# GAP-LAB-CUHK-SZ/gaustudio

Measured on AMD Instinct MI355X. Metric: Mpixels/s fwd+bwd @1M Gaussians 1920x1080, higher is better.
Workload: dtype f32; 1 GPU; C3: 1M synthetic Gaussians, 1920x1080, SH degree 3, fwd+bwd (colour+depth+median+opacity consumed); gaussians=1000000, width=1920, height=1080, sh_degree=3, tiles=8160, views_per_rank=1, loss=colour + depth + median + opacity gradients consumed, camera=static (the same view every step), parallelism=single GPU

## Files before the change

### gaustudio_amd/csrc/gsr_kernels_bwd.hip

```cpp
#include "gsr_internal.h"
#include "gsr_bwd_timing.h"

namespace gsr {

__device__ __constant__ float bSH_C0 = 0.28209479177387814f;
__device__ __constant__ float bSH_C1 = 0.4886025119029199f;
__device__ __constant__ float bSH_C2[5] = {1.0925484305920792f, -1.0925484305920792f, 0.31539156525252005f,
                                            -1.0925484305920792f, 0.5462742152960396f};
__device__ __constant__ float bSH_C3[7] = {-0.5900435899266435f, 2.890611442640554f, -0.4570457994644658f,
                                            0.3731763325901154f, -0.4570457994644658f, 1.445305721320277f,
                                            -0.5900435899266435f};

#define GSR_DPP_ADD(v, ctrl) v += __int_as_float(__builtin_amdgcn_update_dpp(0, __float_as_int(v), ctrl, 0xF, 0xF, true))
#define GSR_DPP_OF(v, ctrl) __int_as_float(__builtin_amdgcn_update_dpp(0, __float_as_int(v), ctrl, 0xF, 0xF, true))
__device__ __forceinline__ float half_swap_sum(float a, float b)
{
	const auto t = __builtin_amdgcn_permlane32_swap(__float_as_uint(a), __float_as_uint(b), false, false);
	return __uint_as_float(t[0]) + __uint_as_float(t[1]);
}
__device__ __forceinline__ float row_swap_sum(float p, float q)
{
	const auto t = __builtin_amdgcn_permlane16_swap(__float_as_uint(p), __float_as_uint(q), false, false);
	return __uint_as_float(t[0]) + __uint_as_float(t[1]);
}
// ... 194 lines not shown
	const bool any_bg = __ballot(bg_dot != 0.f) != 0ull;
	float T_ = T_final;
	float S = 0.f;

	int wmax = lc;
#pragma unroll
	for (int o = 32; o > 0; o >>= 1) wmax = max(wmax, __shfl_xor(wmax, o, 64));
	wmax = __builtin_amdgcn_readfirstlane(wmax);
	if (lane == 0) s_max[wv] = wmax;
	__syncthreads();
	const int bmax = max(max(s_max[0], s_max[1]), max(s_max[2], s_max[3]));

	for (int i = bmax + tid; !FLAGS && i < (int)(range.y - range.x); i += GSR_BWD_THREADS) {
		const uint32_t id = point_list[range.x + i];
		const uint4 q3 = recs[id].q3;
		float4* dst = reinterpret_cast<float4*>(rows + (size_t)(goff[id] + gs_row_in_rect(q3.x, q3.y, (q3.z >> GSR_Q3Z_DEAD_SHIFT) & 15u, tx, ty)) * GSR_ROW_STRIDE);
		dst[0] = make_float4(0.f, 0.f, 0.f, 0.f);
		dst[1] = make_float4(0.f, 0.f, 0.f, 0.f);
		dst[2] = make_float4(0.f, 0.f, 0.f, 0.f);
	}
	float2* slab = s_slab[wv];
	float* plane = s_plane[wv];
	const int srec = tid >> 2, spart = tid & 3;
	auto load_id = [&](int t) -> uint32_t {
		return (t > 0 && srec < min(GSR_BWD_BATCH, t)) ? point_list[range.x + (uint32_t)(t - 1 - srec)] : 0u;
	};
	auto load_part = [&](int t, uint32_t id) -> float4 {
		float4 v = make_float4(0.f, 0.f, 0.f, 0.f);
		if (t > 0 && srec < min(GSR_BWD_BATCH, t)) {
			v = reinterpret_cast<const float4*>(recs + id)[spart];
			if (spart == 3) v.w = __uint_as_float(goff[id]);
		}
		return v;
	};
	uint32_t id_next = load_id(bmax - GSR_BWD_BATCH);
	float4 part_cur = load_part(bmax, load_id(bmax));
	for (int top = bmax; top > 0; top -= GSR_BWD_BATCH) {
		const int cnt = min(GSR_BWD_BATCH, top);
		__syncthreads();
		if (srec < cnt) {
			if (spart == 0) sA[srec] = part_cur;
			else if (spart == 1) sB[srec] = part_cur;
			else if (spart == 2) sC[srec] = part_cur;
			else {
				const uint32_t q3x = __float_as_uint(part_cur.x), q3y = __float_as_uint(part_cur.y), q3w = __float_as_uint(part_cur.w);
				s_row[srec] = q3w + gs_row_in_rect(q3x, q3y, (__float_as_uint(part_cur.z) >> GSR_Q3Z_DEAD_SHIFT) & 15u, tx, ty);
			}
		}
		const float4 part_next = load_part(top - GSR_BWD_BATCH, id_next);
		id_next = load_id(top - 2 * GSR_BWD_BATCH);
		for (int i = tid; i < 4 * GSR_BWD_BATCH * GSR_PLANE_STRIDE / 4; i += GSR_BWD_THREADS)
			reinterpret_cast<float4*>(&s_plane[0][0])[i] = make_float4(0.f, 0.f, 0.f, 0.f);
		__syncthreads();
		bool hit = false;
		if (lane < cnt && top - 1 - lane < wmax) hit = gs_box_may_touch(sA[lane], sB[lane], fbx, fby, bx1, by1);
		unsigned long long m = __ballot(hit);
		int nu = 0;
		unsigned long long unit_js = 0ull;
		auto pair = [&](const float4 A, const float4 B, const float4 Cc, const int j) {
			const int pos = top - 1 - j;
			const float dx = A.x - pixfx, dy = A.y - pixfy;
			const float power = FMA(A.w * dx, dy, FMA(B.x * dy, dy, (A.z * dx) * dx));
			const float G = gs_exp(power);
			const float a0 = B.y * G;
			const bool live = (pos < lc) & (power <= 0.0f) & (power >= B.w) & (!(a0 < 1.0f / 255.0f));
			if (__ballot(live) == 0ull) return;
			const float Gm = live ? G : 0.f;
			const float alpha = fminf(0.99f, B.y * Gm);
			const float rinv = __builtin_amdgcn_rcpf(1.0f - alpha);
			const float test_T = T_ * rinv;
			const float w = alpha * test_T;
			const float cd = FMA(Cc.x, dLp0, FMA(Cc.y, dLp1, FMA(Cc.z, dLp2, FMA(B.z, dLd, dLo))));
			const float diff = cd - S;
			float dL_dalpha = diff * test_T;
			if (any_bg) {
				asm volatile("");
				dL_dalpha = FMA(-(T_final * rinv), bg_dot, dL_dalpha);
			}
			const float q = Gm * dL_dalpha;
			S = FMA(alpha, diff, S);
			T_ = TSEL ? (live ? test_T : T_) : test_T;
			slab[nu * GSR_SLAB_STRIDE + lane] = make_float2(q, w);
			unit_js |= (unsigned long long)j << (8 * nu);
			nu++;
			if (nu == GSR_BWD_UNITS) {
				__builtin_amdgcn_fence(__ATOMIC_RELEASE, "wavefront");
				__builtin_amdgcn_wave_barrier();
				gs_bwd_phase2(GSR_BWD_UNITS, slab, unit_js, sA, s_tab[wv], fbx, fby, top, plane, lane);
				__builtin_amdgcn_wave_barrier();
				nu = 0;
				unit_js = 0ull;
			}
		};
		if (m) {
			int j0 = __ffsll((long long)m) - 1, j1 = 0;
			m &= m - 1;
			float4 A0 = sA[j0], B0 = sB[j0], C0 = sC[j0], A1, B1, C1;
			while (true) {
				const bool more1 = m != 0ull;
				if (more1) {
					j1 = __ffsll((long long)m) - 1;
					m &= m - 1;
					A1 = sA[j1]; B1 = sB[j1]; C1 = sC[j1];
				}
				pair(A0, B0, C0, j0);
				if (!more1) break;
				const bool more0 = m != 0ull;
				if (more0) {
					j0 = __ffsll((long long)m) - 1;
					m &= m - 1;
					A0 = sA[j0]; B0 = sB[j0]; C0 = sC[j0];
				}
				pair(A1, B1, C1, j1);
				if (!more0) break;
			}
		}
		if (nu > 0) {
			__builtin_amdgcn_fence(__ATOMIC_RELEASE, "wavefront");
			__builtin_amdgcn_wave_barrier();
			gs_bwd_phase2(nu, slab, unit_js, sA, s_tab[wv], fbx, fby, top, plane, lane);
		}
		__syncthreads();
		if (tid < cnt) {
			float v[10];
#pragma unroll
			for (int k = 0; k < 10; k++)
				v[k] = ((s_plane[0][tid * GSR_PLANE_STRIDE + k] + s_plane[1][tid * GSR_PLANE_STRIDE + k]) +
				        s_plane[2][tid * GSR_PLANE_STRIDE + k]) + s_plane[3][tid * GSR_PLANE_STRIDE + k];
			const float4 A = sA[tid], B = sB[tid];
			const float ca = -2.f * A.z, cb = -A.w, cc = -2.f * B.x, op = B.y;
			const float M10 = v[0], M01 = v[1], M20 = v[2], M11 = v[3], M02 = v[4];
			const float ddelx_dx = (float)(0.5 * W), ddely_dy = (float)(0.5 * H);
			const uint32_t my_row = s_row[tid];
			float4* dst = reinterpret_cast<float4*>(rows + (size_t)my_row * GSR_ROW_STRIDE);
			dst[0] = make_float4(-(op * FMA(cb, M01, ca * M10)) * ddelx_dx, -(op * FMA(cb, M10, cc * M01)) * ddely_dy,
			                     -0.5f * op * M20, -0.5f * op * M11);
			dst[1] = make_float4(-0.5f * op * M02, v[5], v[6], v[7]);
			dst[2] = make_float4(v[8], v[9], 0.f, 0.f);
			if (FLAGS) row_flags[my_row] = 1;
		}
		part_cur = part_next;
	}
}

#endif

#define GSR_BWQ_U 4
#ifndef GSR_BWQ_BATCH
#define GSR_BWQ_BATCH 128
#endif
#define GSR_BWQ_HALVES ((GSR_BWQ_BATCH + 63) / 64)
#define GSR_BWQ_LIST (GSR_BWQ_BATCH + 8)
#define GSR_BWQ_SENT GSR_BWQ_BATCH
#define GSR_WAIT_VM0() __builtin_amdgcn_s_waitcnt(0x0F70)
#define GSR_BWQ_QSTRIDE 66

#ifndef GSR_BWQ_WAVES
#define GSR_BWQ_WAVES 4
#endif
template <bool FLAGS, bool TSEL, bool FX, bool CONLY>
__global__ __launch_bounds__(GSR_BWD_THREADS) __attribute__((amdgpu_waves_per_eu(GSR_BWQ_WAVES, GSR_BWQ_WAVES))) void composite_bwd_quarter_kernel(
    int T, int chunk, int gx, int W, int H, const GsBg bgv, const uint2* __restrict__ ranges,
    const uint32_t* __restrict__ point_list, const GsRec* __restrict__ recs, const uint32_t* __restrict__ goff,
    const float* __restrict__ final_T, const uint32_t* __restrict__ n_contrib, const uint32_t* __restrict__ med_pos,
    const float* __restrict__ dL_dpix, const float* __restrict__ dL_dpix_depth, const float* __restrict__ dL_dpix_median,
    const float* __restrict__ dL_dpix_opacity, float* __restrict__ rows, uint8_t* __restrict__ row_flags,
    const GsCtl* __restrict__ ctl)
{
	__shared__ float4 sA[GSR_BWQ_BATCH + 1];
	__shared__ float4 sB[GSR_BWQ_BATCH + 1];
	__shared__ float4 sC[GSR_BWQ_BATCH + 1];
	__shared__ uint32_t s_row[GSR_BWQ_BATCH];
	__shared__ uint16_t s_qmask[GSR_BWQ_BATCH];
	__shared__ __attribute__((aligned(16))) float s_plane[4][GSR_BWQ_BATCH * GSR_PLANE_STRIDE];
	__shared__ __attribute__((aligned(16))) float2 s_slab[4][4 * GSR_BWQ_QSTRIDE];
	__shared__ __attribute__((aligned(16))) uint8_t s_list[4][4][GSR_BWQ_LIST];
	__shared__ int s_max[4];
	if (blockIdx.x == 0 && threadIdx.x == 0 && bgv.flag_dst != nullptr) *bgv.flag_dst = bgv.flag;
	const int tb_lo = (int)bgv.tile_lo, tb_n = (int)min(bgv.tile_hi, (uint32_t)T) - tb_lo;
	const int local = (blockIdx.x & 7) * chunk + (blockIdx.x >> 3);
	const int tile = bgv.tile_order ? ((int)blockIdx.x < T ? (int)bgv.tile_order[blockIdx.x] : T) : tb_lo + local;
	if ((!bgv.tile_order && ((int)(blockIdx.x >> 3) >= chunk || local >= tb_n)) || tile >= T) return;
	if ((uint32_t)tile < bgv.tile_lo || (uint32_t)tile >= bgv.tile_hi) return;
	const int tid = threadIdx.x;
	const int lane = tid & 63, wv = tid >> 6, qd = lane >> 4;
	TM_DECL
	const int tx = tile % gx, ty = tile / gx;
	const int lx = ((wv & 1) << 3) + ((qd & 1) << 2) + (lane & 3);
	const int ly = ((wv >> 1) << 3) + ((qd >> 1) << 2) + ((lane >> 2) & 3);
	const int px = tx * GSR_BLOCK_X + lx, py = ty * GSR_BLOCK_Y + ly;
	const bool inside = px < W && py < H;
	const float pixfx = (float)px, pixfy = (float)py;
	const float fbx = (float)(tx * GSR_BLOCK_X + ((wv & 1) << 3)), fby = (float)(ty * GSR_BLOCK_Y + ((wv >> 1) << 3));
	const uint2 range = ranges[tile];
	const bool have_qmask = __builtin_amdgcn_readfirstlane(ctl->has_qmask) != 0u;
	const uint16_t* __restrict__ qmask = gs_qmask_ptr(point_list, __builtin_amdgcn_readfirstlane(ctl->num_binned));

	const size_t sidx = (size_t)tile * GSR_TILE_PIX + (wv << 6) + ((ly & 7) << 3) + (lx & 7);
	const float T_final = inside ? final_T[sidx] : 0.f;
	const int lc = inside ? (int)n_contrib[sidx] : 0;
	float dLp0 = 0.f, dLp1 = 0.f, dLp2 = 0.f, dLd = 0.f, dLo = 0.f, dLm = 0.f;
	uint32_t mpos = 0u;
	if (inside) {
		const size_t HW = (size_t)H * W;
		const size_t pix_id = (size_t)W * py + px;
		if (dL_dpix) {
			dLp0 = dL_dpix[pix_id];
			dLp1 = dL_dpix[HW + pix_id];
			dLp2 = dL_dpix[2 * HW + pix_id];
		}
		if (!CONLY) {
			if (dL_dpix_depth) dLd = dL_dpix_depth[pix_id];
			if (dL_dpix_median) dLm = dL_dpix_median[pix_id];
			if (dL_dpix_opacity) dLo = dL_dpix_opacity[pix_id];
			mpos = med_pos[sidx];
		}
	}
	float2* slab = s_slab[wv];
	float* plane = s_plane[wv];
	const int u2 = (lane >> 2) & 3, r2 = lane & 3;
	float4 g_pix[4];
	float g_op[4];
	{
		float4* tmp = reinterpret_cast<float4*>(slab);
		tmp[2 * lane] = make_float4(dLp0, dLp1, dLp2, dLd);
		if (!CONLY) tmp[2 * lane + 1] = make_float4(dLo, 0.f, 0.f, 0.f);
		__builtin_amdgcn_fence(__ATOMIC_RELEASE, "wavefront");
		__builtin_amdgcn_wave_barrier();
#pragma unroll
		for (int sx = 0; sx < 4; sx++) {
			const int pl = (qd << 4) + (r2 << 2) + sx;
			const float4 gp = tmp[2 * pl];
			const float c0 = gp.x, c1 = gp.y, c2 = gp.z, c3 = gp.w;
			g_pix[sx] = make_float4(r2 == 0 ? c0 : r2 == 1 ? c1 : r2 == 2 ? c2 : c3, r2 == 0 ? c1 : r2 == 1 ? c0 : r2 == 2 ? c3 : c2,
			                        r2 == 0 ? c2 : r2 == 1 ? c3 : r2 == 2 ? c0 : c1, r2 == 0 ? c3 : r2 == 1 ? c2 : r2 == 2 ? c1 : c0);
			g_op[sx] = CONLY ? 0.f : tmp[2 * pl + 1].x;
		}
		__builtin_amdgcn_wave_barrier();
#pragma unroll
		for (int sx = 0; sx < 4; sx++) asm volatile("" : "+v"(g_pix[sx].x), "+v"(g_pix[sx].y), "+v"(g_pix[sx].z), "+v"(g_pix[sx].w));
	}
	const float y2 = fby + (float)(((qd >> 1) << 2) + r2), x2 = fbx + (float)((qd & 1) << 2);
	const float bg0 = bgv.dptr ? bgv.dptr[0] : bgv.host[0], bg1 = bgv.dptr ? bgv.dptr[1] : bgv.host[1], bg2 = bgv.dptr ? bgv.dptr[2] : bgv.host[2];
	const float bg_dot = FMA(bg2, dLp2, FMA(bg1, dLp1, FMA(bg0, dLp0, 0.f)));
	const bool any_bg = __ballot(bg_dot != 0.f) != 0ull;
	float T_ = T_final;
	float S = 0.f;

	int qmax = lc;
	qmax = max(qmax, __shfl_xor(qmax, 1, 64));
	qmax = max(qmax, __shfl_xor(qmax, 2, 64));
	qmax = max(qmax, __shfl_xor(qmax, 4, 64));
	qmax = max(qmax, __shfl_xor(qmax, 8, 64));
	const int qm0 = __builtin_amdgcn_readlane(qmax, 0), qm1 = __builtin_amdgcn_readlane(qmax, 16);
	const int qm2 = __builtin_amdgcn_readlane(qmax, 32), qm3 = __builtin_amdgcn_readlane(qmax, 48);
	const int wmax = max(max(qm0, qm1), max(qm2, qm3));
	if (lane == 0) s_max[wv] = wmax;
	TM(0)
	if (tid < 3) (tid == 0 ? sA : tid == 1 ? sB : sC)[GSR_BWQ_SENT] = make_float4(0.f, 0.f, 0.f, 0.f);
	__syncthreads();
	const int bmax = max(max(s_max[0], s_max[1]), max(s_max[2], s_max[3]));
	TM(1)

	const int srec = tid >> 2, spart = tid & 3;
	const uint32_t* __restrict__ tile_list = point_list + range.x;
	const uint32_t* __restrict__ mask_words = have_qmask ? reinterpret_cast<const uint32_t*>(qmask) : point_list;
	auto list_pos = [&](int t, int h) -> uint32_t {
		return (uint32_t)max(t - 1 - (srec + 64 * h), 0);
	};
	auto word_ptr = [&](int t, int h, uint32_t id) -> const uint32_t* {
		return spart == 2 ? mask_words + ((range.x + list_pos(t, h)) >> 1) : goff + id;
	};
	uint32_t id_next[GSR_BWQ_HALVES];
	float4 part[GSR_BWQ_HALVES];
#pragma unroll
	for (int h = 0; h < GSR_BWQ_HALVES; h++) {
		part[h] = make_float4(0.f, 0.f, 0.f, 0.f);
		id_next[h] = 0u;
	}
	if (bmax > 0) {
		uint32_t id_cur[GSR_BWQ_HALVES];
#pragma unroll
		for (int h = 0; h < GSR_BWQ_HALVES; h++) {
			id_cur[h] = tile_list[list_pos(bmax, h)];
			id_next[h] = tile_list[list_pos(bmax - GSR_BWQ_BATCH, h)];
		}
#pragma unroll
		for (int h = 0; h < GSR_BWQ_HALVES; h++) {
			part[h] = reinterpret_cast<const float4*>(recs + id_cur[h])[spart];
			if (spart >= 2) part[h].w = __uint_as_float(*word_ptr(bmax, h, id_cur[h]));
		}
	}
	for (int i = bmax + tid; !FLAGS && i < (int)(range.y - range.x); i += GSR_BWD_THREADS) {
		const uint32_t id = tile_list[i];
		const uint4 q3 = recs[id].q3;
		float4* dst = reinterpret_cast<float4*>(rows + (size_t)(goff[id] + gs_row_in_rect(q3.x, q3.y, (q3.z >> GSR_Q3Z_DEAD_SHIFT) & 15u, tx, ty)) * GSR_ROW_STRIDE);
		dst[0] = make_float4(0.f, 0.f, 0.f, 0.f);
		dst[1] = make_float4(0.f, 0.f, 0.f, 0.f);
		dst[2] = make_float4(0.f, 0.f, 0.f, 0.f);
	}
	GSR_WAIT_VM0();
	TM(2)
	const uint8_t* my_list = &s_list[wv][qd][0];
	const char* recA = reinterpret_cast<const char*>(sA);
	const char* recB = reinterpret_cast<const char*>(sB);
	const char* recC = reinterpret_cast<const char*>(sC);
	float2* my_slab_w = slab + qd * GSR_BWQ_QSTRIDE + (lane & 15);
	const float4* my_slab_r = reinterpret_cast<const float4*>(slab + qd * GSR_BWQ_QSTRIDE + u2 * 16 + r2 * 4);

	for (int top = bmax; top > 0; top -= GSR_BWQ_BATCH) {
		const int cnt = min(GSR_BWQ_BATCH, top);
		TM(3)
		__syncthreads();
		TM(4)
#pragma unroll
		for (int h = 0; h < GSR_BWQ_HALVES; h++) {
			const int sr = srec + 64 * h;
			if (sr < cnt) {
				if (spart == 0) sA[sr] = part[h];
				else if (spart == 1) {
					float* b = reinterpret_cast<float*>(&sB[sr]);
					*reinterpret_cast<float2*>(b) = make_float2(part[h].x, part[h].y);
					b[2] = part[h].z;
					reinterpret_cast<float2*>(&sC[sr])[1] = make_float2(part[h].w, 0.f);
				} else if (spart == 2) {
					reinterpret_cast<float*>(&sB[sr])[3] = part[h].x;
					*reinterpret_cast<float2*>(&sC[sr]) = make_float2(part[h].y, part[h].z);
					s_qmask[sr] = (uint16_t)(__float_as_uint(part[h].w) >> (16u * ((range.x + (uint32_t)(top - 1 - sr)) & 1u)));
				} else {
					const uint32_t q3x = __float_as_uint(part[h].x), q3y = __float_as_uint(part[h].y), q3z = __float_as_uint(part[h].z);
					s_row[sr] = __float_as_uint(part[h].w) + gs_row_in_rect(q3x, q3y, (q3z >> GSR_Q3Z_DEAD_SHIFT) & 15u, tx, ty);
				}
			}
		}
		TM(5)
#pragma unroll
		for (int h = 0; h < GSR_BWQ_HALVES; h++) {
			part[h] = reinterpret_cast<const float4*>(recs + id_next[h])[spart];
			if (spart >= 2) part[h].w = __uint_as_float(*word_ptr(top - GSR_BWQ_BATCH, h, id_next[h]));
		}
#pragma unroll
		for (int h = 0; h < GSR_BWQ_HALVES; h++) id_next[h] = tile_list[list_pos(top - 2 * GSR_BWQ_BATCH, h)];
		float zero = 0.f;
		uint32_t ss = GSR_BWQ_SENT * 0x01010101u;
		asm volatile("" : "+v"(zero), "+v"(ss));
		for (int i = tid; i < 4 * GSR_BWQ_BATCH * GSR_PLANE_STRIDE / 4; i += GSR_BWD_THREADS)
			reinterpret_cast<float4*>(&s_plane[0][0])[i] = make_float4(zero, zero, zero, zero);
		if (lane < 4 * GSR_BWQ_LIST / 16) {
			reinterpret_cast<uint4*>(&s_list[wv][0][0])[lane] = make_uint4(ss, ss, ss, ss);
		}
		TM(6)
		__syncthreads();
		TM(7)
		if (mpos != 0u && dLm != 0.f && (uint32_t)top >= mpos && (uint32_t)top - mpos < (uint32_t)cnt)
			atomicAdd(&plane[((uint32_t)top - mpos) * GSR_PLANE_STRIDE + 7], dLm);
		int c0 = 0, c1 = 0, c2 = 0, c3 = 0;
#define GSR_APPEND(QQ, CNT)                                                                                          \
	{                                                                                                                \
		const bool h_ = (mk >> (QQ)) & 1u;                                                                           \
		const unsigned long long bm = __ballot(h_);                                                                  \
		const int pos_ = CNT + (int)__builtin_amdgcn_mbcnt_hi((uint32_t)(bm >> 32), __builtin_amdgcn_mbcnt_lo((uint32_t)bm, 0u)); \
		if (h_) s_list[wv][QQ][pos_] = (uint8_t)jl;                                                                  \
		CNT += __popcll(bm);                                                                                         \
	}
#pragma unroll
		for (int h = 0; h < GSR_BWQ_HALVES; h++) {
			const int jl = lane + 64 * h;
			if (64 * h >= cnt) break;
			uint32_t mk = 0;
			if (jl < cnt) {
				if (have_qmask) {
					const uint32_t m16 = (uint32_t)s_qmask[jl] >> (8 * (wv >> 1) + 2 * (wv & 1));
					mk = (m16 & 3u) | ((m16 >> 2) & 12u);
				} else {
					float4 q1 = sB[jl];
					q1.w = sC[jl].z;
					mk = gs_quarter_mask<2>(sA[jl], q1, fbx, fby, 0xfu);
				}
				const int pos = top - 1 - jl;
				mk &= (pos < qm0 ? 1u : 0u) | (pos < qm1 ? 2u : 0u) | (pos < qm2 ? 4u : 0u) | (pos < qm3 ? 8u : 0u);
			}
			GSR_APPEND(0, c0)
			GSR_APPEND(1, c1)
			GSR_APPEND(2, c2)
			GSR_APPEND(3, c3)
		}
#undef GSR_APPEND
		__builtin_amdgcn_wave_barrier();
		TM(8)
		const int n = max(max(c0, c1), max(c2, c3));
		const int my_cnt = qd == 0 ? c0 : qd == 1 ? c1 : qd == 2 ? c2 : c3;
		struct Rec { float4 A, B; float2 C; float pcut; };
		auto fetch = [&](const uint32_t j) -> Rec {
			Rec r;
			r.A = *reinterpret_cast<const float4*>(recA + j * 16);
			r.B = *reinterpret_cast<const float4*>(recB + j * 16);
			if (FX) {
				r.C = *reinterpret_cast<const float2*>(recC + j * 16);
				r.pcut = 0.f;
			} else {
				float4 c = *reinterpret_cast<const float4*>(recC + j * 16);
				asm volatile("" : "+v"(c.w));
				r.C = make_float2(c.x, c.y);
				r.pcut = c.z;
			}
			return r;
		};
		auto step = [&](const Rec& rc, const uint32_t j, const int st) {
			const float4 A = rc.A, B = rc.B;
			const float3 Cc = make_float3(B.w, rc.C.x, rc.C.y);
			const int pos = top - 1 - (int)j;
			const float dx = A.x - pixfx, dy = A.y - pixfy;
			const float power = FMA(A.w * dx, dy, FMA(B.x * dy, dy, (A.z * dx) * dx));
			float G, a0;
			bool live;
			if (!FX) {
				G = gs_exp(power);
				a0 = B.y * G;
				live = (pos < lc) & (power <= 0.0f) & (power >= rc.pcut) & (!(a0 < 1.0f / 255.0f));
			} else {
				G = gs_exp_hw(power);
				a0 = B.y * G;
				live = (pos < lc) & (power <= 0.0f) & (!(a0 < 1.0f / 255.0f));
			}
			const float Gm = live ? G : 0.f;
			const float alpha = fminf(0.99f, B.y * Gm);
			const float rinv = __builtin_amdgcn_rcpf(1.0f - alpha);
			const float test_T = T_ * rinv;
			const float w = alpha * test_T;
			const float cd = FMA(Cc.x, dLp0, FMA(Cc.y, dLp1, FMA(Cc.z, dLp2, CONLY ? 0.f : FMA(B.z, dLd, dLo))));
			const float diff = cd - S;
			float dL_dalpha = diff * test_T;
			if (any_bg) {
				asm volatile("");
				dL_dalpha = FMA(-(T_final * rinv), bg_dot, dL_dalpha);
			}
			const float q = Gm * dL_dalpha;
			S = FMA(alpha, diff, S);
			T_ = TSEL ? (live ? test_T : T_) : test_T;
			my_slab_w[16 * st] = make_float2(q, w);
		};
		float pn0 = 0.f, pn1 = 0.f, pn2 = 0.f, t0 = 0.f, t1 = 0.f, t2 = 0.f;
		float* pn_dst = plane;
		bool pn_act = false;
		const bool r2_hi = (r2 & 2) != 0;
		auto turn_read = [&](const int qq) {
			if (pn_act & (qd == qq)) {
				t0 = pn_dst[0];
				t1 = pn_dst[4];
				if (!r2_hi) t2 = pn_dst[8];
			}
		};
		auto turn_write = [&](const int qq) {
			if (pn_act & (qd == qq)) {
				pn_dst[0] = t0 + pn0;
				pn_dst[4] = t1 + pn1;
				if (!r2_hi) pn_dst[8] = t2 + pn2;
			}
		};
		uint32_t pk = *reinterpret_cast<const uint32_t*>(my_list);
		for (int i = 0; i < n; i += GSR_BWQ_U) {
			const uint32_t cur = pk;
			pk = *reinterpret_cast<const uint32_t*>(my_list + i + GSR_BWQ_U);
			__builtin_amdgcn_sched_barrier(0);
			turn_read(0); step(fetch(cur & 0xffu), cur & 0xffu, 0); turn_write(0);
			turn_read(1); step(fetch((cur >> 8) & 0xffu), (cur >> 8) & 0xffu, 1); turn_write(1);
			turn_read(2); step(fetch((cur >> 16) & 0xffu), (cur >> 16) & 0xffu, 2); turn_write(2);
			turn_read(3); step(fetch(cur >> 24), cur >> 24, 3); turn_write(3);
			__builtin_amdgcn_fence(__ATOMIC_RELEASE, "wavefront");
			__builtin_amdgcn_wave_barrier();
			{
				const bool act = i + u2 < my_cnt;
				const uint32_t j = act ? (cur >> (8 * u2)) & 0xffu : 0u;
				const float2 ctr = *reinterpret_cast<const float2*>(recA + j * 16);
				const float4 v01 = my_slab_r[0], v23 = my_slab_r[1];
				const float dy = ctr.y - y2, X = ctr.x - x2;
				const float qv[4] = {v01.x, v01.z, v23.x, v23.z}, wv_[4] = {v01.y, v01.w, v23.y, v23.w};
				float S0 = 0.f, a0 = 0.f, a2 = 0.f, a5 = 0.f, a6 = 0.f, a7 = 0.f, a8 = 0.f, a9 = 0.f;
#pragma unroll
				for (int sx = 0; sx < 4; sx++) {
					const float dx = X - (float)sx;
					const float t = qv[sx] * dx;
					S0 += qv[sx];
					a0 += t;
					a2 = FMA(t, dx, a2);
					if (!CONLY) a5 = FMA(wv_[sx], g_op[sx], a5);
					a6 = FMA(wv_[sx], g_pix[sx].x, a6);
					a7 = FMA(wv_[sx], g_pix[sx].y, a7);
					a8 = FMA(wv_[sx], g_pix[sx].z, a8);
					a9 = FMA(wv_[sx], g_pix[sx].w, a9);
				}
				a5 += S0;
				float a1 = dy * S0, a3 = dy * a0;
				float a4 = dy * a1;
				GSR_DPP_ADD(a0, 0xB1); GSR_DPP_ADD(a1, 0xB1); GSR_DPP_ADD(a2, 0xB1); GSR_DPP_ADD(a3, 0xB1); GSR_DPP_ADD(a4, 0xB1);
				GSR_DPP_ADD(a5, 0xB1);
				GSR_DPP_ADD(a0, 0x4E); GSR_DPP_ADD(a1, 0x4E); GSR_DPP_ADD(a2, 0x4E); GSR_DPP_ADD(a3, 0x4E); GSR_DPP_ADD(a4, 0x4E);
				GSR_DPP_ADD(a5, 0x4E);
				const float k1 = a6 + GSR_DPP_OF(a7, 0xB1), k2 = a8 + GSR_DPP_OF(a9, 0xB1);
				const bool lo1 = (r2 & 1) != 0;
				pn0 = r2_hi ? (lo1 ? a3 : a2) : (lo1 ? a1 : a0);
				pn1 = k1 + GSR_DPP_OF(k2, 0x4E);
				pn2 = lo1 ? a5 : a4;
				pn_act = act;
				pn_dst = plane + j * GSR_PLANE_STRIDE + r2;
			}
			__builtin_amdgcn_wave_barrier();
		}
#pragma unroll
		for (int qq = 0; qq < 4; qq++) {
			turn_read(qq);
			turn_write(qq);
		}
		TM(9)
		GSR_WAIT_VM0();
		__syncthreads();
		TM(10)
		for (int fj = tid; fj < cnt; fj += GSR_BWD_THREADS) {
			float v[10];
#pragma unroll
			for (int k = 0; k < 10; k++)
				v[k] = ((s_plane[0][fj * GSR_PLANE_STRIDE + k] + s_plane[1][fj * GSR_PLANE_STRIDE + k]) +
				        s_plane[2][fj * GSR_PLANE_STRIDE + k]) + s_plane[3][fj * GSR_PLANE_STRIDE + k];
			const float4 A = sA[fj], B = sB[fj];
			const float ca = -2.f * A.z, cb = -A.w, cc = -2.f * B.x, op = B.y;
			const float M10 = v[0], M01 = v[1], M20 = v[2], M11 = v[3], M02 = v[8];
			const float ddelx_dx = (float)(0.5 * W), ddely_dy = (float)(0.5 * H);
			const uint32_t my_row = s_row[fj];
			float4* dst = reinterpret_cast<float4*>(rows + (size_t)my_row * GSR_ROW_STRIDE);
			dst[0] = make_float4(-(op * FMA(cb, M01, ca * M10)) * ddelx_dx, -(op * FMA(cb, M10, cc * M01)) * ddely_dy,
			                     -0.5f * op * M20, -0.5f * op * M11);
			dst[1] = make_float4(-0.5f * op * M02, v[9], v[4], v[5]);
			dst[2] = make_float4(v[6], v[7], 0.f, 0.f);
			if (FLAGS) row_flags[my_row] = 1;
		}
		TM(11)
	}
	TM_END
}

__global__ void bwd_selftest_kernel(const float* __restrict__ in, uint32_t* __restrict__ out)
{
	const float one = in[0];
	const float r = __builtin_amdgcn_rcpf(one - in[1]);
	uint32_t ok = (__float_as_uint(r) == 0x3f800000u) ? 1u : 0u;
	const float t = 0.37f * in[0];
	if (t * r == t) ok |= 2u;
	out[0] = ok;
	out[1] = __float_as_uint(r);
}
void launch_bwd_selftest(const float* in, uint32_t* out, hipStream_t s)
{
	hipLaunchKernelGGL(bwd_selftest_kernel, dim3(1), dim3(1), 0, s, in, out);
}

__global__ __launch_bounds__(256) void band_classes_kernel(int P, const int* __restrict__ radii, const GsRec* __restrict__ recs, int split,
                                                           int* __restrict__ first, int* __restrict__ second)
{
	const int idx = blockIdx.x * 256 + threadIdx.x;
	if (idx >= P) return;
	const bool vis = radii[idx] > 0;
	const bool c1 = vis && (int)(recs[idx].q3.y >> 16) <= split;
	if (first != nullptr) first[idx] = c1 ? 1 : 0;
	if (second != nullptr) second[idx] = (vis && !c1) ? 1 : 0;
}
void launch_band_classes(int P, const int* radii, const GsRec* recs, int split, int* first, int* second, hipStream_t s)
{
	hipLaunchKernelGGL(band_classes_kernel, dim3((P + 255) / 256), dim3(256), 0, s, P, radii, recs, split, first, second);
}

__device__ __forceinline__ uint32_t gs_work_class(uint32_t m)
{
	if (m < 4u) return m;
	const int e = 31 - __clz((int)m);
	return (uint32_t)(4 * (e - 1)) + ((m >> (e - 2)) & 3u);
}
__global__ __launch_bounds__(256) void tile_work_kernel(int T, const uint32_t* __restrict__ n_contrib, uint32_t* __restrict__ work)
{
	const int tile = blockIdx.x * 4 + (threadIdx.x >> 6), lane = threadIdx.x & 63;
	if (tile >= T) return;
	const uint4 v = reinterpret_cast<const uint4*>(n_contrib + (size_t)tile * GSR_TILE_PIX)[lane];
	uint32_t m = max(max(v.x, v.y), max(v.z, v.w));
#pragma unroll
	for (int o = 32; o > 0; o >>= 1) m = max(m, (uint32_t)__shfl_xor((int)m, o, 64));
	if (lane == 0) work[tile] = m;
}
__global__ __launch_bounds__(1024) void tile_order_kernel(int T, const uint32_t* __restrict__ work, uint32_t* __restrict__ order)
{
	__shared__ uint32_t s_cnt[128], s_cur[128];
	const int tid = threadIdx.x;
	if (tid < 128) s_cnt[tid] = 0u;
	__syncthreads();
	for (int t = tid; t < T; t += 1024) atomicAdd(&s_cnt[gs_work_class(work[t])], 1u);
	__syncthreads();
	if (tid == 0) {
		uint32_t run = 0;
		for (int c = 127; c >= 0; c--) { s_cur[c] = run; run += s_cnt[c]; }
	}
	__syncthreads();
	for (int t = tid; t < T; t += 1024) order[atomicAdd(&s_cur[gs_work_class(work[t])], 1u)] = (uint32_t)t;
}
void launch_tile_order(int T, const uint32_t* n_contrib, uint32_t* tile_work, uint32_t* tile_order, hipStream_t s)
{
	hipLaunchKernelGGL(tile_work_kernel, dim3((T + 3) / 4), dim3(256), 0, s, T, n_contrib, tile_work);
	hipLaunchKernelGGL(tile_order_kernel, dim3(1), dim3(1024), 0, s, T, tile_work, tile_order);
}

void launch_composite_bwd(const ImgLayout& il, int W, int H, const GsBg& bg, const uint2* ranges,
                          const uint32_t* point_list, const GsRec* recs, const uint32_t* goff, const float* final_T,
                          const uint32_t* n_contrib, const uint32_t* med_pos, const float* dL_dpix, const float* dL_dpix_depth,
                          const float* dL_dpix_median, const float* dL_dpix_opacity, float* rows, uint8_t* row_flags,
                          const GsCtl* ctl, int variant, hipStream_t s)
{
	const int tb_n = (int)std::min(bg.tile_hi, (uint32_t)il.T) - (int)bg.tile_lo;
	const int chunk = bg.tile_order ? (il.T + 7) / 8 : std::max(1, (tb_n + 7) / 8);
	const bool tsel = (variant & 1) != 0, wave_lists = (variant & 2) != 0;
	const bool fx = (variant & 8) != 0;
	const bool flags = row_flags != nullptr;
#define GSR_LAUNCH_CB(...)                                                                                         \
	hipLaunchKernelGGL((__VA_ARGS__), dim3(chunk * 8), dim3(GSR_BWD_THREADS), 0, s, il.T, chunk, il.gx, W, H, bg,  \
	                   ranges, point_list, recs, goff, final_T, n_contrib, med_pos, dL_dpix, dL_dpix_depth, dL_dpix_median, \
	                   dL_dpix_opacity, rows, row_flags, ctl)
#ifdef GSR_AB_VARIANTS
	if (wave_lists) {
		if (flags) { if (tsel) GSR_LAUNCH_CB(composite_bwd_kernel<true, true>); else GSR_LAUNCH_CB(composite_bwd_kernel<true, false>); }
		else { if (tsel) GSR_LAUNCH_CB(composite_bwd_kernel<false, true>); else GSR_LAUNCH_CB(composite_bwd_kernel<false, false>); }
	} else
#else
	(void)wave_lists;
#endif
	if (dL_dpix_depth == nullptr && dL_dpix_median == nullptr && dL_dpix_opacity == nullptr && !tsel) {
		if (fx) { if (flags) GSR_LAUNCH_CB(composite_bwd_quarter_kernel<true, false, true, true>); else GSR_LAUNCH_CB(composite_bwd_quarter_kernel<false, false, true, true>); }
		else { if (flags) GSR_LAUNCH_CB(composite_bwd_quarter_kernel<true, false, false, true>); else GSR_LAUNCH_CB(composite_bwd_quarter_kernel<false, false, false, true>); }
	} else if (fx) {
		if (flags) { if (tsel) GSR_LAUNCH_CB(composite_bwd_quarter_kernel<true, true, true, false>); else GSR_LAUNCH_CB(composite_bwd_quarter_kernel<true, false, true, false>); }
		else { if (tsel) GSR_LAUNCH_CB(composite_bwd_quarter_kernel<false, true, true, false>); else GSR_LAUNCH_CB(composite_bwd_quarter_kernel<false, false, true, false>); }
	} else {
		if (flags) { if (tsel) GSR_LAUNCH_CB(composite_bwd_quarter_kernel<true, true, false, false>); else GSR_LAUNCH_CB(composite_bwd_quarter_kernel<true, false, false, false>); }
		else { if (tsel) GSR_LAUNCH_CB(composite_bwd_quarter_kernel<false, true, false, false>); else GSR_LAUNCH_CB(composite_bwd_quarter_kernel<false, false, false, false>); }
	}
#undef GSR_LAUNCH_CB
}

template <int D, bool FLAGS>
__global__ __launch_bounds__(256) void preprocess_bwd_kernel(
    int P, int M, const float* __restrict__ means3D, const int* __restrict__ radii, const float* __restrict__ shs,
    const float* __restrict__ scales, const float* __restrict__ rotations, float scale_modifier,
    const float* __restrict__ cov3D_precomp, const GsCam* __restrict__ cam, int W, int H, float tan_fovx,
    float tan_fovy, float h_x, float h_y, int sh_vec4, int act, const GsRec* __restrict__ recs,
    const uint32_t* __restrict__ goff, const float* __restrict__ rows, const uint8_t* __restrict__ row_flags,
    float* __restrict__ dL_dmean2D, float* __restrict__ dL_dopacity, float* __restrict__ dL_dcolor,
    float* __restrict__ dL_dmeans, float* __restrict__ dL_dcov, float* __restrict__ dL_dsh,
    float* __restrict__ dL_dscale, float* __restrict__ dL_drot, int mask_colors, int cls_mode, int cls_split)
{
	const int idx = blockIdx.x * 256 + threadIdx.x;
	bool mine = true;
	if (cls_mode != 0) {
		const bool v_ = idx < P && radii[idx] > 0;
		const int rmaxy = v_ ? (int)(recs[idx].q3.y >> 16) : 0;
		mine = ((!v_ || rmaxy <= cls_split) ? 1 : 2) == cls_mode;
		if (__ballot(mine && idx < P) == 0ull) return;
// ... 617 lines not shown
```

Before: 2262 Mpixels/s.

## Store pre-scaled 16-bit list entries and specialize backward walk on background

The per-quad gaussian index lists now hold 16-bit entries already multiplied by 16 bytes, so the inner loop addresses shared records directly with no per-step multiply. The depth test becomes a single compare against a running threshold. The background branch is hoisted out of the hot loop by instantiating the walk twice. The DPP reductions in the second phase are restructured to select operands before the butterfly adds, which cuts the number of cross-lane ops. In exchange the list uses twice as much LDS, it fills with a loop, and the code grows larger.

```diff
diff --git a/gaustudio_amd/csrc/gsr_kernels_bwd.hip b/gaustudio_amd/csrc/gsr_kernels_bwd.hip
--- a/gaustudio_amd/csrc/gsr_kernels_bwd.hip
+++ b/gaustudio_amd/csrc/gsr_kernels_bwd.hip
@@ -370,6 +370,8 @@
 #define GSR_BWQ_HALVES ((GSR_BWQ_BATCH + 63) / 64)
 #define GSR_BWQ_LIST (GSR_BWQ_BATCH + 8)
 #define GSR_BWQ_SENT GSR_BWQ_BATCH
+#define GSR_BWQ_ENTRY(j) ((uint32_t)(j) << 4)
+template <bool B> struct GsBool { static constexpr bool value = B; };
 #define GSR_WAIT_VM0() __builtin_amdgcn_s_waitcnt(0x0F70)
 #define GSR_BWQ_QSTRIDE 66
 
@@ -392,7 +394,7 @@
 	__shared__ uint16_t s_qmask[GSR_BWQ_BATCH];
 	__shared__ __attribute__((aligned(16))) float s_plane[4][GSR_BWQ_BATCH * GSR_PLANE_STRIDE];
 	__shared__ __attribute__((aligned(16))) float2 s_slab[4][4 * GSR_BWQ_QSTRIDE];
-	__shared__ __attribute__((aligned(16))) uint8_t s_list[4][4][GSR_BWQ_LIST];
+	__shared__ __attribute__((aligned(16))) uint16_t s_list[4][4][GSR_BWQ_LIST];
 	__shared__ int s_max[4];
 	if (blockIdx.x == 0 && threadIdx.x == 0 && bgv.flag_dst != nullptr) *bgv.flag_dst = bgv.flag;
 	const int tb_lo = (int)bgv.tile_lo, tb_n = (int)min(bgv.tile_hi, (uint32_t)T) - tb_lo;
@@ -401,7 +403,7 @@
 	if ((!bgv.tile_order && ((int)(blockIdx.x >> 3) >= chunk || local >= tb_n)) || tile >= T) return;
 	if ((uint32_t)tile < bgv.tile_lo || (uint32_t)tile >= bgv.tile_hi) return;
 	const int tid = threadIdx.x;
-	const int lane = tid & 63, wv = tid >> 6, qd = lane >> 4;
+	const int lane = tid & 63, wv = __builtin_amdgcn_readfirstlane(tid >> 6), qd = lane >> 4;
 	TM_DECL
 	const int tx = tile % gx, ty = tile / gx;
 	const int lx = ((wv & 1) << 3) + ((qd & 1) << 2) + (lane & 3);
@@ -519,7 +521,8 @@
 	}
 	GSR_WAIT_VM0();
 	TM(2)
-	const uint8_t* my_list = &s_list[wv][qd][0];
+	const uint16_t* my_list = &s_list[wv][qd][0];
+	int thr16 = (bmax - 1 - lc) * 16;
 	const char* recA = reinterpret_cast<const char*>(sA);
 	const char* recB = reinterpret_cast<const char*>(sB);
 	const char* recC = reinterpret_cast<const char*>(sC);
@@ -560,13 +563,13 @@
 #pragma unroll
 		for (int h = 0; h < GSR_BWQ_HALVES; h++) id_next[h] = tile_list[list_pos(top - 2 * GSR_BWQ_BATCH, h)];
 		float zero = 0.f;
-		uint32_t ss = GSR_BWQ_SENT * 0x01010101u;
+		uint32_t ss = GSR_BWQ_ENTRY(GSR_BWQ_SENT) * 0x00010001u;
 		asm volatile("" : "+v"(zero), "+v"(ss));
 		for (int i = tid; i < 4 * GSR_BWQ_BATCH * GSR_PLANE_STRIDE / 4; i += GSR_BWD_THREADS)
 			reinterpret_cast<float4*>(&s_plane[0][0])[i] = make_float4(zero, zero, zero, zero);
-		if (lane < 4 * GSR_BWQ_LIST / 16) {
-			reinterpret_cast<uint4*>(&s_list[wv][0][0])[lane] = make_uint4(ss, ss, ss, ss);
-		}
+		static_assert((4 * GSR_BWQ_LIST * sizeof(uint16_t)) % 16 == 0, "a wave's lists are filled 16 B at a time");
+		for (int i = lane; i < (int)(4 * GSR_BWQ_LIST * sizeof(uint16_t) / 16); i += 64)
+			reinterpret_cast<uint4*>(&s_list[wv][0][0])[i] = make_uint4(ss, ss, ss, ss);
 		TM(6)
 		__syncthreads();
 		TM(7)
@@ -578,7 +581,7 @@
 		const bool h_ = (mk >> (QQ)) & 1u;                                                                           \
 		const unsigned long long bm = __ballot(h_);                                                                  \
 		const int pos_ = CNT + (int)__builtin_amdgcn_mbcnt_hi((uint32_t)(bm >> 32), __builtin_amdgcn_mbcnt_lo((uint32_t)bm, 0u)); \
-		if (h_) s_list[wv][QQ][pos_] = (uint8_t)jl;                                                                  \
+		if (h_) s_list[wv][QQ][pos_] = (uint16_t)GSR_BWQ_ENTRY(jl);                                                  \
 		CNT += __popcll(bm);                                                                                         \
 	}
 #pragma unroll
@@ -609,25 +612,25 @@
 		const int n = max(max(c0, c1), max(c2, c3));
 		const int my_cnt = qd == 0 ? c0 : qd == 1 ? c1 : qd == 2 ? c2 : c3;
 		struct Rec { float4 A, B; float2 C; float pcut; };
-		auto fetch = [&](const uint32_t j) -> Rec {
+		auto fetch = [&](const uint32_t e) -> Rec {
 			Rec r;
-			r.A = *reinterpret_cast<const float4*>(recA + j * 16);
-			r.B = *reinterpret_cast<const float4*>(recB + j * 16);
+			r.A = *reinterpret_cast<const float4*>(recA + e);
+			r.B = *reinterpret_cast<const float4*>(recB + e);
 			if (FX) {
-				r.C = *reinterpret_cast<const float2*>(recC + j * 16);
+				r.C = *reinterpret_cast<const float2*>(recC + e);
 				r.pcut = 0.f;
 			} else {
-				float4 c = *reinterpret_cast<const float4*>(recC + j * 16);
+				float4 c = *reinterpret_cast<const float4*>(recC + e);
 				asm volatile("" : "+v"(c.w));
 				r.C = make_float2(c.x, c.y);
 				r.pcut = c.z;
 			}
 			return r;
 		};
-		auto step = [&](const Rec& rc, const uint32_t j, const int st) {
+		auto step = [&](const Rec& rc, const uint32_t e, const int st, auto BG) {
 			const float4 A = rc.A, B = rc.B;
 			const float3 Cc = make_float3(B.w, rc.C.x, rc.C.y);
-			const int pos = top - 1 - (int)j;
+			const bool in_front = (int)e > thr16;
 			const float dx = A.x - pixfx, dy = A.y - pixfy;
 			const float power = FMA(A.w * dx, dy, FMA(B.x * dy, dy, (A.z * dx) * dx));
 			float G, a0;
@@ -635,11 +638,11 @@
 			if (!FX) {
 				G = gs_exp(power);
 				a0 = B.y * G;
-				live = (pos < lc) & (power <= 0.0f) & (power >= rc.pcut) & (!(a0 < 1.0f / 255.0f));
+				live = in_front & (power <= 0.0f) & (power >= rc.pcut) & (!(a0 < 1.0f / 255.0f));
 			} else {
 				G = gs_exp_hw(power);
 				a0 = B.y * G;
-				live = (pos < lc) & (power <= 0.0f) & (!(a0 < 1.0f / 255.0f));
+				live = in_front & (power <= 0.0f) & (!(a0 < 1.0f / 255.0f));
 			}
 			const float Gm = live ? G : 0.f;
 			const float alpha = fminf(0.99f, B.y * Gm);
@@ -649,10 +652,7 @@
 			const float cd = FMA(Cc.x, dLp0, FMA(Cc.y, dLp1, FMA(Cc.z, dLp2, CONLY ? 0.f : FMA(B.z, dLd, dLo))));
 			const float diff = cd - S;
 			float dL_dalpha = diff * test_T;
-			if (any_bg) {
-				asm volatile("");
-				dL_dalpha = FMA(-(T_final * rinv), bg_dot, dL_dalpha);
-			}
+			if (decltype(BG)::value) dL_dalpha = FMA(-(T_final * rinv), bg_dot, dL_dalpha);
 			const float q = Gm * dL_dalpha;
 			S = FMA(alpha, diff, S);
 			T_ = TSEL ? (live ? test_T : T_) : test_T;
@@ -676,32 +676,25 @@
 				if (!r2_hi) pn_dst[8] = t2 + pn2;
 			}
 		};
-		uint32_t pk = *reinterpret_cast<const uint32_t*>(my_list);
-		for (int i = 0; i < n; i += GSR_BWQ_U) {
-			const uint32_t cur = pk;
-			pk = *reinterpret_cast<const uint32_t*>(my_list + i + GSR_BWQ_U);
-			__builtin_amdgcn_sched_barrier(0);
-			turn_read(0); step(fetch(cur & 0xffu), cur & 0xffu, 0); turn_write(0);
-			turn_read(1); step(fetch((cur >> 8) & 0xffu), (cur >> 8) & 0xffu, 1); turn_write(1);
-			turn_read(2); step(fetch((cur >> 16) & 0xffu), (cur >> 16) & 0xffu, 2); turn_write(2);
-			turn_read(3); step(fetch(cur >> 24), cur >> 24, 3); turn_write(3);
-			__builtin_amdgcn_fence(__ATOMIC_RELEASE, "wavefront");
-			__builtin_amdgcn_wave_barrier();
+		const uint32_t sel2 = 0x0c0c0000u | ((2u * u2 + 1u) << 8) | (2u * u2);
+		auto phase2 = [&](const uint2 cur, const int i) {
 			{
 				const bool act = i + u2 < my_cnt;
-				const uint32_t j = act ? (cur >> (8 * u2)) & 0xffu : 0u;
-				const float2 ctr = *reinterpret_cast<const float2*>(recA + j * 16);
+				const uint32_t e = act ? (FX ? __builtin_amdgcn_perm(cur.y, cur.x, sel2) : (uint32_t)my_list[i + u2]) : 0u;
+				const float2 ctr = *reinterpret_cast<const float2*>(recA + e);
 				const float4 v01 = my_slab_r[0], v23 = my_slab_r[1];
 				const float dy = ctr.y - y2, X = ctr.x - x2;
 				const float qv[4] = {v01.x, v01.z, v23.x, v23.z}, wv_[4] = {v01.y, v01.w, v23.y, v23.w};
-				float S0 = 0.f, a0 = 0.f, a2 = 0.f, a5 = 0.f, a6 = 0.f, a7 = 0.f, a8 = 0.f, a9 = 0.f;
+				float S0 = qv[0], a0 = qv[0] * X, a2 = FMA(a0, X, 0.f), a5 = 0.f, a6 = 0.f, a7 = 0.f, a8 = 0.f, a9 = 0.f;
 #pragma unroll
 				for (int sx = 0; sx < 4; sx++) {
 					const float dx = X - (float)sx;
-					const float t = qv[sx] * dx;
-					S0 += qv[sx];
-					a0 += t;
-					a2 = FMA(t, dx, a2);
+					if (sx > 0) {
+						const float t = qv[sx] * dx;
+						S0 += qv[sx];
+						a0 += t;
+						a2 = FMA(t, dx, a2);
+					}
 					if (!CONLY) a5 = FMA(wv_[sx], g_op[sx], a5);
 					a6 = FMA(wv_[sx], g_pix[sx].x, a6);
 					a7 = FMA(wv_[sx], g_pix[sx].y, a7);
@@ -711,20 +704,40 @@
 				a5 += S0;
 				float a1 = dy * S0, a3 = dy * a0;
 				float a4 = dy * a1;
-				GSR_DPP_ADD(a0, 0xB1); GSR_DPP_ADD(a1, 0xB1); GSR_DPP_ADD(a2, 0xB1); GSR_DPP_ADD(a3, 0xB1); GSR_DPP_ADD(a4, 0xB1);
-				GSR_DPP_ADD(a5, 0xB1);
-				GSR_DPP_ADD(a0, 0x4E); GSR_DPP_ADD(a1, 0x4E); GSR_DPP_ADD(a2, 0x4E); GSR_DPP_ADD(a3, 0x4E); GSR_DPP_ADD(a4, 0x4E);
-				GSR_DPP_ADD(a5, 0x4E);
+				const bool lo1 = (r2 & 1) != 0;
+				const float b01 = (lo1 ? a1 : a0) + GSR_DPP_OF(lo1 ? a0 : a1, 0xB1);
+				const float b23 = (lo1 ? a3 : a2) + GSR_DPP_OF(lo1 ? a2 : a3, 0xB1);
+				const float b45 = (lo1 ? a5 : a4) + GSR_DPP_OF(lo1 ? a4 : a5, 0xB1);
 				const float k1 = a6 + GSR_DPP_OF(a7, 0xB1), k2 = a8 + GSR_DPP_OF(a9, 0xB1);
-				const bool lo1 = (r2 & 1) != 0;
-				pn0 = r2_hi ? (lo1 ? a3 : a2) : (lo1 ? a1 : a0);
+				pn0 = (r2_hi ? b23 : b01) + GSR_DPP_OF(r2_hi ? b01 : b23, 0x4E);
 				pn1 = k1 + GSR_DPP_OF(k2, 0x4E);
-				pn2 = lo1 ? a5 : a4;
+				pn2 = b45 + GSR_DPP_OF(b45, 0x4E);
 				pn_act = act;
-				pn_dst = plane + j * GSR_PLANE_STRIDE + r2;
-			}
-			__builtin_amdgcn_wave_barrier();
-		}
+				pn_dst = plane + (e >> 4) * GSR_PLANE_STRIDE + r2;
+			}
+		};
+		uint2 pk = *reinterpret_cast<const uint2*>(my_list);
+#define GSR_BWQ_WALK(BG)                                                                                                    \
+		for (int i = 0; i < n; i += GSR_BWQ_U) {                                                                            \
+			const uint2 cur = pk;                                                                                           \
+			pk = *reinterpret_cast<const uint2*>(my_list + i + GSR_BWQ_U);                                                  \
+			__builtin_amdgcn_sched_barrier(0);                                                                              \
+			turn_read(0); step(fetch(cur.x & 0xffffu), cur.x & 0xffffu, 0, BG); turn_write(0);                              \
+			turn_read(1); step(fetch(cur.x >> 16), cur.x >> 16, 1, BG); turn_write(1);                                      \
+			turn_read(2); step(fetch(cur.y & 0xffffu), cur.y & 0xffffu, 2, BG); turn_write(2);                              \
+			turn_read(3); step(fetch(cur.y >> 16), cur.y >> 16, 3, BG); turn_write(3);                                      \
+			__builtin_amdgcn_fence(__ATOMIC_RELEASE, "wavefront");                                                          \
+			__builtin_amdgcn_wave_barrier();                                                                                \
+			phase2(cur, i);                                                                                                 \
+			__builtin_amdgcn_wave_barrier();                                                                                \
+		}
+		if (any_bg) {
+			GSR_BWQ_WALK(GsBool<true>{})
+		} else {
+			GSR_BWQ_WALK(GsBool<false>{})
+		}
+#undef GSR_BWQ_WALK
+		thr16 -= GSR_BWQ_BATCH * 16;
 #pragma unroll
 		for (int qq = 0; qq < 4; qq++) {
 			turn_read(qq);
```

After: 2300 Mpixels/s (median of 6 runs). 1.02x the previous value.
